# GEM3D/pressurePoissonSolver

Hardware: NVIDIA B200
Metric: fp64 GMG V-cycle DOF/s (higher is better)
Workload: dtype f64

## Files before the change

pressurepoissonsolver_b200/csrc/patch3d32.cuh:

```cuda
#pragma once

namespace tgpu
{
template <int D, int N, int MODE>
__device__ __forceinline__ double gamma_entry(const PatchMeta &pm, int p, int s, int m, const FaceVals<D, N, MODE> &fv)
{
	const int ty = pm.nbr_type[s];
	if (ty == NBR_NONE) return 0.0;
	if (ty == NBR_NORMAL) {
		const double a = fv.get(p, pm.parent_idx, pm.orth_on_parent, s, m);
		const double b = fv.get(pm.nbr_idx[s][0], pm.nbr_parent[s], pm.nbr_orth[s], s ^ 1, m);
		return 0.5 * a + 0.5 * b;
	}
	return iface_gamma<D, N, MODE>(pm, p, s, m, fv);
}

constexpr int    C32_THREADS = 512, C32_ROW = 34, C32_PL = 32 * C32_ROW, C32_TILE = 16 * C32_PL;
constexpr int    C32_FV = 65;
constexpr size_t smooth3d32c_smem_bytes() { return sizeof(double) * (C32_TILE + 2 * 1024 + 1024 + 16 * 128 + 16 * 64); }
static_assert(32 * C32_FV <= 1024 + 16 * 128, "the face-vector staging aliases the interface-value buffers of sweeps from a zero guess");
__device__ __forceinline__ unsigned cluster_ctarank()
{
	unsigned r;
	asm volatile("mov.u32 %0, %%cluster_ctarank;\n" : "=r"(r));
	return r;
}
__device__ __forceinline__ void cluster_sync_all()
{
	asm volatile("barrier.cluster.arrive.release.aligned;\nbarrier.cluster.wait.acquire.aligned;\n" ::: "memory");
}
__device__ __forceinline__ double ld_dsmem(const double *local, unsigned rank)
{
	unsigned a = (unsigned) __cvta_generic_to_shared(local), ra;
	double   v;
	asm volatile("mapa.shared::cluster.u32 %0, %1, %2;\n" : "=r"(ra) : "r"(a), "r"(rank));
	asm volatile("ld.shared::cluster.f64 %0, [%1];\n" : "=d"(v) : "r"(ra) : "memory");
	return v;
}
template <bool PROLONG>
__device__ __noinline__ double gamma_entry32(const PatchMeta *__restrict__ meta, int p, int s, int m, const double *__restrict__ F,
                                             const double *__restrict__ uc)
{
	const FaceVals<3, 32, PROLONG ? FV_PROLONG : FV_PLAIN> fv{F, uc, meta};
	return gamma_entry(meta[p], p, s, m, fv);
}
struct __align__(16) GDesc32 {
	unsigned a0, b0, a1, b1;
	double   c;
	int      flags, pad;
};
struct GPatch32 {
	GDesc32 d[6];
	int     neu, pad[3];
};
template <bool PROLONG>
__device__ __forceinline__ void make_gdesc32(const PatchMeta &pm, int p, int s, GPatch32 &out)
{
	GDesc32 & d  = out.d[s];
	const int ty = pm.nbr_type[s];
	const int ax = s >> 1;
	const int st = (ax == 0) ? 1 : (ax == 1 ? 32 : 1024);
	d.a0 = d.b0 = ((unsigned) p * 6 + s) * 1024;
	d.a1 = d.b1 = 0;
	d.c         = (ty == NBR_NONE) ? 0.0 : 2.0 * pm.inv_h2;
	int fl      = GD_SA | GD_SB | GD_WB;
	if (ty == NBR_NORMAL) {
		d.b0 = ((unsigned) pm.nbr_idx[s][0] * 6 + (s ^ 1)) * 1024;
		if (PROLONG) {
			const int o = pm.orth_on_parent, qp = pm.nbr_parent[s], qo = pm.nbr_orth[s];
			if (o >= 0) d.a1 = (unsigned) pm.parent_idx * 32768 + 16 * ((o & 1) + 32 * ((o >> 1) & 1) + 1024 * ((o >> 2) & 1)) + ((s & 1) ? 15 * st : 0);
			else d.a1 = (unsigned) pm.parent_idx * 32768 + ((s & 1) ? 31 * st : 0), fl &= ~GD_SA;
			if (qp < 0) d.b1 = d.a1, fl = (fl & ~(GD_SB | GD_WB)) | ((fl & GD_SA) ? GD_SB : 0);
			else if (qo >= 0) d.b1 = (unsigned) qp * 32768 + 16 * ((qo & 1) + 32 * ((qo >> 1) & 1) + 1024 * ((qo >> 2) & 1)) + ((s & 1) ? 0 : 15 * st);
			else d.b1 = (unsigned) qp * 32768 + ((s & 1) ? 0 : 31 * st), fl &= ~GD_SB;
		}
	} else if (ty > NBR_NORMAL) {
		fl = GD_SA | GD_SB | GD_WB | GD_SLOW;
	}
	d.flags = fl;
}
template <bool PROLONG> struct SideGamma32 {
	double a0, a1, b0, b1;
	template <int AX>
	__device__ __forceinline__ void issue(const GDesc32 &d, int m, int lo, int hi, const double *__restrict__ F, const double *__restrict__ uc)
	{
		constexpr int A = (AX == 0) ? 32 : 1, B = (AX == 2) ? 32 : 1024;
		const uint4   o = *reinterpret_cast<const uint4 *>(&d);
		a0 = __ldg(F + o.x + m);
		b0 = __ldg(F + o.y + m);
		a1 = b1 = 0.0;
		if (PROLONG) {
			const int fl = d.flags, sa = fl & GD_SA, sb = (fl >> 1) & 1;
			a1 = __ldg(uc + o.z + ((lo >> sa) * A + (hi >> sa) * B));
			b1 = __ldg(uc + o.w + ((lo >> sb) * A + (hi >> sb) * B));
		}
	}
	__device__ __forceinline__ double finish(const GDesc32 &d, const PatchMeta *__restrict__ meta, int p, int s, int m, const double *__restrict__ F,
	                                         const double *__restrict__ uc) const
	{
		const double c  = d.c;
		const int    fl = d.flags;
		double       g  = c * (0.5 * (a0 + a1) + 0.5 * (b0 + ((fl & GD_WB) ? b1 : 0.0)));
		if (fl & GD_SLOW) g = c * gamma_entry32<PROLONG>(meta, p, s, m, F, uc);
		return g;
	}
};

template <bool ZERO_GUESS, bool EMIT, bool PROLONG, bool WRITE_U, bool HALO = false>
__global__ void __cluster_dims__(2, 1, 1) __launch_bounds__(C32_THREADS, 1)
smooth3d32c_kernel(const PatchMeta *__restrict__ meta, int p0, int P, const double *__restrict__ f, double *__restrict__ u,
                   const double *__restrict__ Fin, double *__restrict__ Fout, const double *__restrict__ tri,
                   const double *__restrict__ uc, HaloSync hs = HaloSync{}, int skip_neumann = 0)
{
	constexpr int N = 32, ROW = C32_ROW, PL = C32_PL, M = N * N, NC = N * N * N;
	extern __shared__ __align__(16) double S[];
	double *       X    = S + C32_TILE;
	double *       GZ   = X + 2 * M;
	double *       GXY  = GZ + M;
	double *       EX   = GXY + 16 * 128;
	double *       FV   = GZ;
	const int      t = threadIdx.x, lane = t & 31, w = t >> 5;
	const unsigned rank = cluster_ctarank();
	const int      z    = rank == 0 ? w : N - 1 - w;
	const int      sz   = rank == 0 ? 4 : 5;
	const int      ncl = gridDim.x / 2, npatch = P - p0;
	double *       gxy  = GXY + w * 128;
	const int      mf   = lane + N * z;
	Mags<N>        mg;
	mg.load();
	pdl_launch_dependents();
	pdl_wait();
	if (!ZERO_GUESS) if (HALO) halo_push<3, 32>(hs, meta);
	int g = blockIdx.x / 2;
	bool halo_ok = false;
	constexpr int                   MW = (int) (sizeof(PatchMeta) / sizeof(double));
	__shared__ __align__(16) double metaS[MW];
	__shared__ GPatch32             GD[2];
	auto describe = [&](const PatchMeta &pm, int q, int slot) {
		if (lane == 31 && w < 6) make_gdesc32<PROLONG>(pm, q, w, GD[slot]);
		if (lane == 31 && w == 6) GD[slot].neu = pm.neumann;
	};
	const int zlo = t & 31, zhi = t >> 5;
	if (!ZERO_GUESS && g < npatch) {
		const int p = p0 + g;
		if (HALO) halo_wait_cta(hs, p, halo_ok);
		describe(meta[p], p, 0);
		if (g + ncl < npatch) describe(meta[p + ncl], p + ncl, 1);
		__syncthreads();
		SideGamma32<PROLONG> g6[6];
		g6[0].template issue<0>(GD[0].d[0], mf, lane, z, Fin, uc);
		g6[1].template issue<0>(GD[0].d[1], mf, lane, z, Fin, uc);
		g6[2].template issue<1>(GD[0].d[2], mf, lane, z, Fin, uc);
		g6[3].template issue<1>(GD[0].d[3], mf, lane, z, Fin, uc);
		g6[4].template issue<2>(GD[0].d[sz], t, zlo, zhi, Fin, uc);
		g6[5].template issue<2>(GD[0].d[sz], t + 512, zlo, zhi + 16, Fin, uc);
#pragma unroll
		for (int s = 0; s < 4; s++) gxy[s * 32 + lane] = g6[s].finish(GD[0].d[s], meta, p, s, mf, Fin, uc);
		GZ[t]       = g6[4].finish(GD[0].d[sz], meta, p, sz, t, Fin, uc);
		GZ[t + 512] = g6[5].finish(GD[0].d[sz], meta, p, sz, t + 512, Fin, uc);
		__syncthreads();
	}
	for (int it = 0; g < npatch; g += ncl, it++) {
		const int    p    = p0 + g;
		const bool   next = g + ncl < npatch;
		const int    pn   = p + ncl;
		const double h2   = meta[p].h2;
		double       v[N];
		if (!ZERO_GUESS && t < MW && g + 2 * ncl < npatch) cp_async8(&metaS[t], reinterpret_cast<const double *>(meta + pn + ncl) + t, true);
		if (skip_neumann && (ZERO_GUESS ? meta[p].neumann : GD[it & 1].neu)) {
			if (!ZERO_GUESS) {
				cp_async_wait_all();
				__syncthreads();
				const GPatch32 &gq = GD[(it + 1) & 1];
				if (next) {
					if (HALO) halo_wait_cta(hs, pn, halo_ok);
					SideGamma32<PROLONG> s6[6];
					s6[0].template issue<0>(gq.d[0], mf, lane, z, Fin, uc);
					s6[1].template issue<0>(gq.d[1], mf, lane, z, Fin, uc);
					s6[2].template issue<1>(gq.d[2], mf, lane, z, Fin, uc);
					s6[3].template issue<1>(gq.d[3], mf, lane, z, Fin, uc);
					s6[4].template issue<2>(gq.d[sz], t, zlo, zhi, Fin, uc);
					s6[5].template issue<2>(gq.d[sz], t + 512, zlo, zhi + 16, Fin, uc);
#pragma unroll
					for (int s = 0; s < 4; s++) gxy[s * 32 + lane] = s6[s].finish(gq.d[s], meta, pn, s, mf, Fin, uc);
					GZ[t]       = s6[4].finish(gq.d[sz], meta, pn, sz, t, Fin, uc);
					GZ[t + 512] = s6[5].finish(gq.d[sz], meta, pn, sz, t + 512, Fin, uc);
					if (g + 2 * ncl < npatch) describe(*reinterpret_cast<const PatchMeta *>(metaS), pn + ncl, it & 1);
				}
				__syncthreads();
			}
			cluster_sync_all();
			continue;
		}
		{
			const double *fp = f + (size_t) p * NC + (size_t) z * M + lane;
#pragma unroll
			for (int k = 0; k < N; k++) v[k] = __ldcs(fp + k * N);
			if (next) {
				const double *fn = f + (size_t) pn * NC + (size_t) z * M + lane * 32;
				prefetch_l2(fn);
				prefetch_l2(fn + 16);
			}
			if (!ZERO_GUESS) {
				v[0] -= gxy[64 + lane];
				v[N - 1] -= gxy[96 + lane];
				if (lane == 0 || lane == N - 1) {
					const double *q = gxy + (lane ? 32 : 0);
#pragma unroll
					for (int k = 0; k < N; k++) v[k] -= q[k];
				}
				if (w == 0) {
#pragma unroll
					for (int k = 0; k < N; k++) v[k] -= GZ[lane + N * k];
				}
			}
			Dst2<N, N>::run(v, mg);
			double *col = S + w * PL + lane;
#pragma unroll
			for (int k = 0; k < N; k++) col[k * ROW] = v[k];
		}
		__syncwarp();
		double2 *rowp = reinterpret_cast<double2 *>(S + w * PL + lane * ROW);
		{
#pragma unroll
			for (int j = 0; j < N / 2; j++) {
				const double2 d = rowp[j];
				v[2 * j]        = d.x;
				v[2 * j + 1]    = d.y;
			}
			Dst2<N, N>::run(v, mg);
#pragma unroll
			for (int j = 0; j < N / 2; j++) rowp[j] = make_double2(v[2 * j], v[2 * j + 1]);
		}
		if (!ZERO_GUESS) cp_async_wait_all();
		__syncthreads();
		if (HALO && !ZERO_GUESS && next) halo_wait_cta(hs, pn, halo_ok);
		SideGamma32<PROLONG> gm[3];
		const GPatch32 &     gp = GD[(it + 1) & 1];
		if (!ZERO_GUESS && next) {
			gm[0].template issue<0>(gp.d[0], mf, lane, z, Fin, uc);
			gm[1].template issue<0>(gp.d[1], mf, lane, z, Fin, uc);
			gm[2].template issue<1>(gp.d[2], mf, lane, z, Fin, uc);
			if (g + 2 * ncl < npatch) describe(*reinterpret_cast<const PatchMeta *>(metaS), pn + ncl, it & 1);
		}
		const double hsc = h2 * (4.0 / (N * N));
		double *     Xo = X + (it & 1) * M;
#pragma unroll
		for (int q = 0; q < 2; q++) {
			const int     ky = w + 16 * q;
			const double *zp = S + ky * ROW + lane;
			const double *tb = tri + ky * N + lane;
			double        rho = 0.0;
#pragma unroll
			for (int j = 0; j < 16; j++) {
				const double a = __ldg(tb + j * M);
				const double r = zp[j * PL] * (hsc * a);
				rho            = (j == 0) ? r : fma(-a, rho, r);
				const_cast<double *>(zp)[j * PL] = rho;
			}
			Xo[ky * N + lane] = rho;
		}
		if (!ZERO_GUESS && next) {
#pragma unroll
			for (int s = 0; s < 3; s++) gxy[s * 32 + lane] = gm[s].finish(gp.d[s], meta, pn, s, mf, Fin, uc);
			gm[0].template issue<1>(gp.d[3], mf, lane, z, Fin, uc);
			gm[1].template issue<2>(gp.d[sz], t, zlo, zhi, Fin, uc);
			gm[2].template issue<2>(gp.d[sz], t + 512, zlo, zhi + 16, Fin, uc);
		}
		cluster_sync_all();
#pragma unroll
		for (int q = 0; q < 2; q++) {
			const int     ky = w + 16 * q;
			double *      zp = S + ky * ROW + lane;
			const double *tb = tri + ky * N + lane;
			const double  a15 = __ldg(tb + 15 * M), kap = __ldg(tb + 16 * M);
			double        y   = kap * fma(-a15, ld_dsmem(Xo + ky * N + lane, rank ^ 1), zp[15 * PL]);
			zp[15 * PL]       = y;
#pragma unroll
			for (int j = 14; j >= 0; j--) {
				y          = fma(-__ldg(tb + j * M), y, zp[j * PL]);
				zp[j * PL] = y;
			}
		}
		if (!ZERO_GUESS && next) {
			gxy[96 + lane] = gm[0].finish(gp.d[3], meta, pn, 3, mf, Fin, uc);
			GZ[t]          = gm[1].finish(gp.d[sz], meta, pn, sz, t, Fin, uc);
			GZ[t + 512]    = gm[2].finish(gp.d[sz], meta, pn, sz, t + 512, Fin, uc);
		}
		__syncthreads();
		constexpr bool FACE_TAIL = ZERO_GUESS && !WRITE_U;
		if (!FACE_TAIL || w == 0) {
			{
#pragma unroll
				for (int j = 0; j < N / 2; j++) {
					const double2 d = rowp[j];
					v[2 * j]        = d.x;
					v[2 * j + 1]    = d.y;
				}
				Dst3<N, N>::run(v, mg);
#pragma unroll
				for (int j = 0; j < N / 2; j++) rowp[j] = make_double2(v[2 * j], v[2 * j + 1]);
			}
			__syncwarp();
			{
				const double *col = S + w * PL + lane;
#pragma unroll
				for (int k = 0; k < N; k++) v[k] = col[k * ROW];
				Dst3<N, N>::run(v, mg);
				if (WRITE_U) {
					double *up = u + (size_t) p * NC + (size_t) z * M + lane;
#pragma unroll
					for (int k = 0; k < N; k++) __stcs(up + k * N, v[k]);
				}
				if (EMIT) {
					double *Fp = Fout + (size_t) p * 6 * M;
					Fp[2 * M + mf] = v[0];
					Fp[3 * M + mf] = v[N - 1];
					if (w == 0) {
						double *Fz = Fp + sz * M + lane;
#pragma unroll
						for (int k = 0; k < N; k++) Fz[N * k] = v[k];
// ... 17 lines not shown
				E               = fma(mg.sinq(2 * j + 1), d.x, E);
				O               = fma((2 * j + 1 == N - 1) ? 0.5 : mg.sinq(2 * j + 2), d.y, O);
			}
			const int vi = 4 * (w - 1);
			FV[lane * C32_FV + vi]     = E + O;
			FV[lane * C32_FV + vi + 1] = E - O;
			const double *col = S + w * PL + lane;
			E = O = 0.0;
#pragma unroll
			for (int k = 0; k < N; k += 2) {
				E = fma(mg.sinq(k + 1), col[k * ROW], E);
				O = fma((k + 1 == N - 1) ? 0.5 : mg.sinq(k + 2), col[(k + 1) * ROW], O);
			}
			FV[lane * C32_FV + vi + 2] = E + O;
			FV[lane * C32_FV + vi + 3] = E - O;
		}
		if (FACE_TAIL) {
			__syncthreads();
			const int vec = (w - 1) * 32 + lane;
			if ((w == 1 || w == 2) && vec < 60) {
#pragma unroll
				for (int j = 0; j < N; j++) v[j] = FV[j * C32_FV + vec];
				Dst3<N, N>::run(v, mg);
				const int lp = 1 + (vec >> 2), kind = vec & 3;
				const int zz = rank == 0 ? lp : N - 1 - lp;
				double *  Fq = Fout + (size_t) p * 6 * M + kind * M + N * zz;
#pragma unroll
				for (int j = 0; j < N / 2; j++) *reinterpret_cast<double2 *>(Fq + 2 * j) = make_double2(v[2 * j], v[2 * j + 1]);
			}
		}
		__syncwarp();
	}
	cluster_sync_all();
	if (!ZERO_GUESS) if (HALO) halo_finish(hs);
}

__global__ void __launch_bounds__(TGPU_THREADS)
smooth3d32n_kernel(const PatchMeta *__restrict__ meta, int p0, int P, const double *__restrict__ f, double *__restrict__ u,
                   const double *__restrict__ Fin, double *__restrict__ Fout, const double *__restrict__ uc,
                   const double *__restrict__ mats, const double *__restrict__ lam, double *__restrict__ scratch, int zero_guess,
                   int emit, int prolong, int write_u, double lam_shift, int only_neumann = 0)
{
	constexpr int N = 32, M = N * N, NC = M * N;
	const int     t = threadIdx.x;
	double *      W = scratch + (size_t) blockIdx.x * NC;
	Mags<N>       mg;
	mg.load();
	pdl_launch_dependents();
	pdl_wait();
	for (int g = blockIdx.x; g < P - p0; g += gridDim.x) {
		const int        p    = p0 + g;
		const PatchMeta &pm   = meta[p];
		const int        neu  = pm.neumann;
		if (only_neumann && !neu) continue;
		const double     cfac = 2.0 * pm.inv_h2, h2 = pm.h2;
		for (int i = t; i < NC; i += TGPU_THREADS) W[i] = __ldg(f + (size_t) p * NC + i);
		__syncthreads();
		if (!zero_guess) {
			for (int s = 0; s < 6; s++) {
				if (pm.nbr_type[s] != NBR_NONE) {
					for (int m = t; m < M; m += TGPU_THREADS) {
						const double gm = prolong ? gamma_entry32<true>(meta, p, s, m, Fin, uc) : gamma_entry32<false>(meta, p, s, m, Fin, uc);
						int          c[3];
						face_cell<3, N>(s, m, c);
						W[(c[2] * N + c[1]) * N + c[0]] -= cfac * gm;
					}
				}
// ... 184 lines not shown
```

pressurepoissonsolver_b200/csrc/tgpu.cu:

```cuda
#include <algorithm>
#include <dlfcn.h>
#include <nccl.h>
#include <cmath>
#include <cstdio>
#include <cstdlib>
#include <cstring>
#include <map>
#include <memory>
#include <stdexcept>
#include <string>
#include <vector>

#include "../../include/tgpu.h"
#include "kernels.cuh"
#include "mesh.h"

using namespace tgpu;

extern "C" int tgpu_hierarchy_destroy(tgpu_hier *h);
static thread_local std::string g_last_error;
static int fail(int code, const std::string &msg)
{
	g_last_error = msg;
	return code;
// ... 125 lines not shown
}

struct tgpu_mesh {
	Mesh                       mesh;
	std::vector<HostLevel>     levels;
	std::vector<TgpuLevelDesc> descs;
};

struct tgpu_part {
	Partition                  part;
	std::vector<TgpuLevelDesc> descs;
};

struct PeerDev {
	int    peer = -1;
	size_t send_off = 0, send_n = 0, recv_off = 0, recv_n = 0;
};
struct LevelDev {
	int        P      = 0;
	int64_t    global_P = 0;
	int        slots  = 0;
	bool       distributed = false;
	int        n_interior  = 0;
	cudaEvent_t ev[4] = {nullptr, nullptr, nullptr, nullptr};
	std::vector<PeerDev> peers;
	int32_t *  send_patch = nullptr, *send_side = nullptr, *recv_slot = nullptr, *recv_side = nullptr;
	double *   sendbuf = nullptr, *recvbuf = nullptr;
	size_t     nsend = 0, nrecv = 0;
	size_t     ncells = 0, nface = 0;
	PatchMeta *meta    = nullptr;
	double *   starts  = nullptr;
	double *   spacing = nullptr;
	double *   Fa = nullptr, *Fb = nullptr;
	double *   u = nullptr, *f = nullptr, *r = nullptr;
	bool       has_neumann = false;
	int32_t *  neu_list = nullptr;
	std::vector<int32_t> neu_host;
	bool       p2p = false;
	int32_t *  send_peer = nullptr, *send_ridx = nullptr, *peer_rank = nullptr;
	double **  peerFa = nullptr, **peerFb = nullptr;
	uint64_t **peer_data_flag = nullptr, **peer_ack_flag = nullptr;
	uint64_t * data_flags = nullptr, *ack_flags = nullptr;
	uint64_t * cnt = nullptr;
	unsigned * tickets = nullptr;
	PushDesc * push_desc = nullptr;
	const double *push_uc = nullptr;
};

struct GraphEntry {
	bool    want_faces = false;
	double *faces      = nullptr;
	const double *  f;
	double *        u;
	TgpuCycleOpts   opts;
	cudaGraphExec_t exec;
	int64_t         kernels;
};

struct tgpu_hier {
	tgpu_ctx *            ctx = nullptr;
	int                   D = 0, N = 0;
	std::vector<LevelDev> levels;
	double *              scratch32 = nullptr;
	double *              cycle_faces = nullptr;
	double *              tri = nullptr;
	double *              mats = nullptr, *lam = nullptr;
// ... 121 lines not shown
}
static int set_smem_attrs_3d16()
{
	TRY((set_smem_attr_3d16<true, true, false, true>()));
	TRY((set_smem_attr_3d16<true, false, false, true>()));
	TRY((set_smem_attr_3d16<true, true, false, false>()));
	TRY((set_smem_attr_3d16<false, true, false, true>()));
	TRY((set_smem_attr_3d16<false, false, false, true>()));
	TRY((set_smem_attr_3d16<false, true, false, false>()));
	TRY((set_smem_attr_3d16<false, true, true, true>()));
	TRY((set_smem_attr_3d16<false, false, true, true>()));
	TRY((set_smem_attr_3d16<false, true, true, false>()));
	return TGPU_OK;
}
template <bool Z, bool E, bool PR, bool W> static int set_smem_attr_2d32()
{
	CU(cudaFuncSetAttribute(smooth2d32_kernel<Z, E, PR, W, false>, cudaFuncAttributeMaxDynamicSharedMemorySize, (int) smooth2d32_smem_bytes()));
	CU(cudaFuncSetAttribute(smooth2d32_kernel<Z, E, PR, W, true>, cudaFuncAttributeMaxDynamicSharedMemorySize, (int) smooth2d32_smem_bytes()));
	return TGPU_OK;
}
static int setup_2d32()
{
	TRY((set_smem_attr_2d32<true, true, false, true>()));
	TRY((set_smem_attr_2d32<true, false, false, true>()));
	TRY((set_smem_attr_2d32<true, true, false, false>()));
	TRY((set_smem_attr_2d32<false, true, false, true>()));
	TRY((set_smem_attr_2d32<false, false, false, true>()));
	TRY((set_smem_attr_2d32<false, true, false, false>()));
	TRY((set_smem_attr_2d32<false, true, true, true>()));
	TRY((set_smem_attr_2d32<false, false, true, true>()));
	TRY((set_smem_attr_2d32<false, true, true, false>()));
	return TGPU_OK;
}
template <bool Z, bool E, bool PR, bool W> static int set_smem_attr_3d32()
{
	CU(cudaFuncSetAttribute(smooth3d32c_kernel<Z, E, PR, W, !Z>, cudaFuncAttributeMaxDynamicSharedMemorySize, (int) smooth3d32c_smem_bytes()));
	return TGPU_OK;
}
static int setup_3d32(tgpu_hier *h)
{
	TRY((set_smem_attr_3d32<true, true, false, true>()));
	TRY((set_smem_attr_3d32<true, false, false, true>()));
	TRY((set_smem_attr_3d32<true, true, false, false>()));
	TRY((set_smem_attr_3d32<false, true, false, true>()));
	TRY((set_smem_attr_3d32<false, false, false, true>()));
	TRY((set_smem_attr_3d32<false, true, false, false>()));
	TRY((set_smem_attr_3d32<false, true, true, true>()));
	TRY((set_smem_attr_3d32<false, false, true, true>()));
	TRY((set_smem_attr_3d32<false, true, true, false>()));
	CU(cudaFuncSetAttribute(apply3d32_tma_kernel<0>, cudaFuncAttributeMaxDynamicSharedMemorySize, (int) apply3d32_tma_smem_bytes()));
	CU(cudaFuncSetAttribute(apply3d32_tma_kernel<1>, cudaFuncAttributeMaxDynamicSharedMemorySize, (int) apply3d32_tma_smem_bytes()));
	CU(cudaFuncSetAttribute(apply3d32_tma_kernel<3>, cudaFuncAttributeMaxDynamicSharedMemorySize, (int) apply3d32_tma_smem_bytes()));
	CU(cudaFuncSetAttribute(face_residual_restrict_big_kernel<3, 32, true>, cudaFuncAttributeMaxDynamicSharedMemorySize, 6 * 1024 * 8));
	CU(cudaFuncSetAttribute(face_residual_restrict_big_kernel<3, 32, false>, cudaFuncAttributeMaxDynamicSharedMemorySize, 6 * 1024 * 8));
	CU(cudaFuncSetAttribute(face_residual_restrict_big_kernel<3, 32, true, true>, cudaFuncAttributeMaxDynamicSharedMemorySize, 6 * 1024 * 8));
	CU(cudaFuncSetAttribute(face_residual_restrict_big_kernel<3, 32, false, true>, cudaFuncAttributeMaxDynamicSharedMemorySize, 6 * 1024 * 8));
	for (const LevelDev &L : h->levels)
		if (L.has_neumann && !h->scratch32) CU(cudaMalloc(&h->scratch32, (size_t) h->ctx->sm_count * 2 * 32768 * sizeof(double)));
	return TGPU_OK;
}
template <int D, int N> static int set_smem_attrs()
{
	const int sb = (int) smooth_smem_bytes<D, N, true>();
	CU(cudaFuncSetAttribute(smooth_kernel<D, N, true, true, false>, cudaFuncAttributeMaxDynamicSharedMemorySize, sb));
	CU(cudaFuncSetAttribute(smooth_kernel<D, N, true, false, false>, cudaFuncAttributeMaxDynamicSharedMemorySize, sb));
	CU(cudaFuncSetAttribute(smooth_kernel<D, N, false, true, false>, cudaFuncAttributeMaxDynamicSharedMemorySize, sb));
	CU(cudaFuncSetAttribute(smooth_kernel<D, N, false, false, false>, cudaFuncAttributeMaxDynamicSharedMemorySize, sb));
	CU(cudaFuncSetAttribute(smooth_kernel<D, N, false, true, true>, cudaFuncAttributeMaxDynamicSharedMemorySize, sb));
	CU(cudaFuncSetAttribute(smooth_kernel<D, N, false, false, true>, cudaFuncAttributeMaxDynamicSharedMemorySize, sb));
	if (D == 3 && N == 16) TRY(set_smem_attrs_3d16());
	CU(cudaFuncSetAttribute(apply_tma_kernel<D, N, 0>, cudaFuncAttributeMaxDynamicSharedMemorySize, (int) apply_tma_smem_bytes<D, N>()));
	CU(cudaFuncSetAttribute(apply_tma_kernel<D, N, 1>, cudaFuncAttributeMaxDynamicSharedMemorySize, (int) apply_tma_smem_bytes<D, N>()));
	CU(cudaFuncSetAttribute(apply_tma_kernel<D, N, 2>, cudaFuncAttributeMaxDynamicSharedMemorySize, (int) apply_tma_smem_bytes<D, N>()));
	CU(cudaFuncSetAttribute(apply_tma_kernel<D, N, 3>, cudaFuncAttributeMaxDynamicSharedMemorySize, (int) apply_tma_smem_bytes<D, N>()));
	return TGPU_OK;
}

static int init_constant_tables()
{
	for (int n : {4, 8, 16, 32}) {
		const int           H = n / 2;
		std::vector<double> fwd((size_t) n * H), inv((size_t) H * n);
// ... 321 lines not shown
		}
		for (size_t m = 0; m < M; m++) {
			const long double mu = (D == 2) ? ll[m] : ll[m % n] + ll[m / n];
			long double       a  = 0.0L;
			for (int j = 0; j < H; j++) {
				const long double d = mu - (j == 0 ? 3.0L : 2.0L);
				a                   = 1.0L / (d - (j == 0 ? 0.0L : a));
				tri[(size_t) j * M + m] = (double) a;
			}
			tri[(size_t) H * M + m] = (double) (1.0L / (1.0L - a * a));
		}
		TRY(dev_upload(&h->tri, tri.data(), tri.size()));
	}
	{
		std::vector<double> mats((size_t) 6 * n * n), lam((size_t) 3 * n);
		auto M = [&](int kind, int k, int j) -> double & { return mats[((size_t) kind * n + k) * n + j]; };
		for (int k = 0; k < n; k++)
			for (int j = 0; j < n; j++) {
				M(0, k, j) = sin(M_PI / n * ((k + 1) * (j + 0.5)));
				M(1, k, j) = (j == n - 1) ? ((k % 2 == 0) ? 0.5 : -0.5) : sin(M_PI / n * ((k + 0.5) * (j + 1)));
				M(2, k, j) = cos(M_PI / n * (k * (j + 0.5)));
				M(3, k, j) = (j == 0) ? 0.5 : cos(M_PI / n * ((k + 0.5) * j));
				M(4, k, j) = cos(M_PI / n * ((k + 0.5) * (j + 0.5)));
				M(5, k, j) = sin(M_PI / n * ((k + 0.5) * (j + 0.5)));
			}
		const double shift[3] = {1.0, 0.0, 0.5};
		for (int t = 0; t < 3; t++)
			for (int k = 0; k < n; k++) lam[(size_t) t * n + k] = -4.0 * pow(sin((k + shift[t]) * M_PI / (2 * n)), 2);
		TRY(dev_upload(&h->mats, mats.data(), mats.size()));
		TRY(dev_upload(&h->lam, lam.data(), lam.size()));
	}
	if (D == 3 && n == 32) TRY(setup_3d32(h.get()));
	else DISPATCH_DN(D, n, TRY((set_smem_attrs<DD, NN>())));
	if (D == 2 && n == 32) TRY(setup_2d32());
	*out = h.release();
	return TGPU_OK;
	API_END
}
extern "C" int tgpu_hierarchy_create(tgpu_ctx *ctx, int D, int n, int nlevels, const TgpuLevelDesc *levels, tgpu_hier **out)
{
	return hierarchy_create_impl(ctx, D, n, nlevels, levels, nullptr, out);
}

extern "C" int tgpu_mesh_partition(tgpu_mesh *m, int n, int rank, int nranks, int min_patches_per_rank, tgpu_part **out)
{
	API_BEGIN
	if (!m || !out) return fail(TGPU_ERR_ARG, "null argument");
	if (n < 2 || (n & 1)) return fail(TGPU_ERR_ARG, "n must be even and >= 2");
	std::unique_ptr<tgpu_part> p(new tgpu_part());
	std::vector<HostLevel>     global = m->mesh.extractLevels(n);
	p->part                           = partitionLevels(global, m->mesh.D, n, rank, nranks, min_patches_per_rank);
	for (const PartLevel &L : p->part.levels) p->descs.push_back(L.local.desc());
	*out = p.release();
	return TGPU_OK;
	API_END
}
extern "C" int tgpu_part_destroy(tgpu_part *p)
{
	delete p;
	return TGPU_OK;
}
extern "C" int tgpu_part_info(const tgpu_part *p, int *nlevels, int *ndist)
{
	if (!p) return fail(TGPU_ERR_ARG, "null partition");
	if (nlevels) *nlevels = (int) p->part.levels.size();
	if (ndist) *ndist = p->part.ndist;
// ... 306 lines not shown
	for (GraphEntry &g : h->graphs) cudaGraphExecDestroy(g.exec);
	h->graphs.clear();
}
extern "C" int tgpu_vec_destroy(tgpu_vec *v);
extern "C" int tgpu_hierarchy_destroy(tgpu_hier *h)
{
	if (!h) return TGPU_OK;
	cudaSetDevice(h->ctx->device);
	if (h->s_in) cudaStreamSynchronize(h->s_in);
	if (h->s_out) cudaStreamSynchronize(h->s_out);
	cudaStreamSynchronize(h->ctx->stream);
	free_graphs(h);
	for (tgpu_vec *v : h->krylov_ws) tgpu_vec_destroy(v);
	tgpu_vec_destroy(h->host_f);
	tgpu_vec_destroy(h->host_u);
	for (int k = 0; k < 2; k++) {
		tgpu_vec_destroy(h->pipe_f[k]);
		tgpu_vec_destroy(h->pipe_u[k]);
		if (h->ev_in[k]) cudaEventDestroy(h->ev_in[k]);
		if (h->ev_cyc[k]) cudaEventDestroy(h->ev_cyc[k]);
		if (h->ev_out[k]) cudaEventDestroy(h->ev_out[k]);
	}
	if (h->s_in) cudaStreamDestroy(h->s_in);
	if (h->s_out) cudaStreamDestroy(h->s_out);
	for (LevelDev &L : h->levels) {
		cudaFree(L.meta);
		cudaFree(L.neu_list);
		cudaFree(L.starts);
		cudaFree(L.spacing);
		if (!L.p2p) {
			cudaFree(L.Fa);
			cudaFree(L.Fb);
		}
		cudaFree(L.send_peer);
		cudaFree(L.send_ridx);
		cudaFree(L.peer_rank);
		cudaFree(L.peerFa);
		cudaFree(L.peerFb);
		cudaFree(L.peer_data_flag);
		cudaFree(L.peer_ack_flag);
		cudaFree(L.cnt);
		cudaFree(L.tickets);
		cudaFree(L.push_desc);
		for (int e = 0; e < 4; e++)
			if (L.ev[e]) cudaEventDestroy(L.ev[e]);
		cudaFree(L.send_patch);
		cudaFree(L.send_side);
		cudaFree(L.recv_slot);
		cudaFree(L.recv_side);
		cudaFree(L.sendbuf);
		cudaFree(L.recvbuf);
		cudaFree(L.u);
		cudaFree(L.f);
		cudaFree(L.r);
	}
	for (void *b : h->ipc_opened) cudaIpcCloseMemHandle(b);
	cudaFree(h->arena);
	cudaFree(h->p2p_abort);
	cudaFree(h->krylov_sc);
	cudaFree(h->mats);
	cudaFree(h->lam);
	cudaFree(h->scratch32);
	cudaFree(h->tri);
	delete h;
	return TGPU_OK;
}
// ... 8 lines not shown
	CU(cudaStreamSynchronize(ctx->stream));
	free_graphs(h);
	for (tgpu_vec *v : h->krylov_ws) tgpu_vec_destroy(v);
	h->krylov_ws.clear();
	tgpu_vec_destroy(h->host_f), h->host_f = nullptr;
	tgpu_vec_destroy(h->host_u), h->host_u = nullptr;
	for (int k = 0; k < 2; k++) {
		tgpu_vec_destroy(h->pipe_f[k]), h->pipe_f[k] = nullptr;
		tgpu_vec_destroy(h->pipe_u[k]), h->pipe_u[k] = nullptr;
	}
	h->pipe_count = 0;
	CU(cudaStreamSynchronize(ctx->stream));
	cudaMemPool_t pool = nullptr;
	CU(cudaDeviceGetDefaultMemPool(&pool, ctx->device));
	CU(cudaMemPoolTrimTo(pool, 0));
	return TGPU_OK;
	API_END
}
extern "C" int tgpu_hierarchy_info(const tgpu_hier *h, int *D, int *n, int *nlevels)
{
	if (!h) return fail(TGPU_ERR_ARG, "null hierarchy");
	if (D) *D = h->D;
	if (n) *n = h->N;
	if (nlevels) *nlevels = (int) h->levels.size();
	return TGPU_OK;
}
extern "C" int tgpu_hierarchy_set_lambda(tgpu_hier *h, double lambda)
{
	if (!h) return fail(TGPU_ERR_ARG, "null argument");
	if (!(lambda == lambda)) return fail(TGPU_ERR_ARG, "tgpu_hierarchy_set_lambda: lambda is NaN");
	h->lambda = lambda;
	if (lambda != 0.0 && is_3d32(h) && !h->scratch32) CU(cudaMalloc(&h->scratch32, (size_t) h->ctx->sm_count * 2 * 32768 * sizeof(double)));
	free_graphs(h);
	return TGPU_OK;
}
extern "C" int tgpu_hierarchy_force_generic_kernels(tgpu_hier *h, int on)
{
	if (!h) return fail(TGPU_ERR_ARG, "null argument");
	h->generic_kernels = on != 0;
	free_graphs(h);
	return TGPU_OK;
}
extern "C" int tgpu_level_npatch(const tgpu_hier *h, int level, int64_t *npatch, int64_t *ncells)
{
	if (!h || level < 0 || level >= (int) h->levels.size()) return fail(TGPU_ERR_ARG, "bad level");
	if (npatch) *npatch = h->levels[level].P;
	if (ncells) *ncells = (int64_t) h->levels[level].ncells;
	return TGPU_OK;
}

extern "C" int tgpu_vec_create(tgpu_hier *h, int level, tgpu_vec **out)
{
	if (!h || !out || level < 0 || level >= (int) h->levels.size()) return fail(TGPU_ERR_ARG, "tgpu_vec_create: bad argument");
	CU(cudaSetDevice(h->ctx->device));
	std::unique_ptr<tgpu_vec> v(new tgpu_vec());
	v->h     = h;
	v->level = level;
	v->n     = h->levels[level].ncells;
	CU(cudaMallocAsync(&v->d, std::max<size_t>(1, v->n) * sizeof(double), h->ctx->stream));
	CU(cudaMemsetAsync(v->d, 0, v->n * sizeof(double), h->ctx->stream));
	*out = v.release();
	return TGPU_OK;
}
extern "C" int tgpu_vec_destroy(tgpu_vec *v)
{
	if (!v) return TGPU_OK;
// ... 279 lines not shown
	if (p1 < 0) p1 = L.P;
	if (p1 <= p0) return hs.push ? fail(TGPU_ERR_ARG, "k_smooth: a launch that pushes faces needs patches") : TGPU_OK;
	if (!emit) write_u = true;
	struct ClampScope {
		tgpu_ctx *c;
		~ClampScope() { c->clamp_resident = false; }
	} clamp_scope{h->ctx};
	h->ctx->clamp_resident = hs.push != nullptr;
	Tag tg(h->ctx, zero_guess ? (write_u ? "smooth_zero_guess" : "smooth_zero_guess_faces")
	                          : (uc ? (write_u ? "smooth_prolong" : "smooth_prolong_faces") : (write_u ? "smooth" : "smooth_faces")),
	       l);
	const bool prolong = uc != nullptr;
	const PatchMeta *meta = L.meta;
	auto generic_smooth = [&](auto dd, auto nn, int only_neumann) {
		constexpr int DD = decltype(dd)::value, NN = decltype(nn)::value;
		using G          = Geo<DD, NN>;
		const int    nblk = (p1 - p0 + G::PPB - 1) / G::PPB;
		const dim3   grid(std::min(nblk, h->ctx->sm_count * smooth_min_blocks<NN>())), block(TGPU_THREADS);
		const size_t sm = smooth_smem_bytes<DD, NN, true>();
		return smooth_variant(zero_guess, emit, prolong, write_u, [&](auto Z, auto E, auto PR, auto) {
			return launch(h->ctx, smooth_kernel<DD, NN, Z, E, PR>, grid, block, sm, meta, p0, p1, f, u, Fin, Fout, (const double *) h->tri, uc,
			              (const double *) h->mats, (const double *) h->lam, h->lambda, only_neumann);
		});
	};
	const bool general = L.has_neumann || h->lambda != 0.0;
	const bool split = !(getenv("TGPU_NEUMANN_SPLIT") && atoi(getenv("TGPU_NEUMANN_SPLIT")) == 0);
	const bool mixed32 = is_3d32(h) && L.has_neumann && h->lambda == 0.0 && !hsp && split;
	if (is_3d32(h) && general) {
		const int nblk = std::min(p1 - p0, h->ctx->sm_count * 2);
		if (!h->scratch32) return fail(TGPU_ERR_ARG, "k_smooth: scratch for the general 32^3 patch solve missing");
		TRY(launch(h->ctx, smooth3d32n_kernel, dim3(nblk), dim3(TGPU_THREADS), 0, (const PatchMeta *) L.meta, p0, p1, f, u, Fin, Fout, uc,
		           (const double *) h->mats, (const double *) h->lam, h->scratch32, (int) zero_guess, (int) emit, (int) (uc != nullptr), (int) write_u, h->lambda,
		           mixed32 ? 1 : 0));
		if (!mixed32) return TGPU_OK;
	}
	if (is_3d32(h)) {
		const dim3   grid(2 * std::min(p1 - p0, h->ctx->sm_count / 2)), block(C32_THREADS);
		const size_t sm    = smooth3d32c_smem_bytes();
		const int    skipn = mixed32 ? 1 : 0;
		return smooth_variant(zero_guess, emit, prolong, write_u, [&](auto Z, auto E, auto PR, auto W) {
			return launch(h->ctx, smooth3d32c_kernel<Z, E, PR, W, !Z>, grid, block, sm, meta, p0, p1, f, u, Fin, Fout, (const double *) h->tri, uc, hs, skipn);
		});
	}
	const bool mixed16 = h->D == 3 && h->N == 16 && !h->generic_kernels && L.has_neumann && h->lambda == 0.0 && !hsp && split;
	if (h->D == 3 && h->N == 16 && !h->generic_kernels && (!general || mixed16)) {
		const int skipn = mixed16 ? 1 : 0;
		static const bool neu_fast = !(getenv("TGPU_NEUMANN_FAST") && atoi(getenv("TGPU_NEUMANN_FAST")) == 0);
		if (mixed16 && neu_fast) {
			TRY(smooth_variant(zero_guess, emit, prolong, write_u, [&](auto Z, auto E, auto PR, auto W) {
				return launch_smooth3d16<Z, E, PR, W>(h, L, p0, p1, f, u, Fin, Fout, uc, HaloSync{}, 0, true);
			}));
		} else if (mixed16) {
			TRY(generic_smooth(std::integral_constant<int, 3>{}, std::integral_constant<int, 16>{}, 1));
		}
		return smooth_variant(zero_guess, emit, prolong, write_u, [&](auto Z, auto E, auto PR, auto W) {
			return launch_smooth3d16<Z, E, PR, W>(h, L, p0, p1, f, u, Fin, Fout, uc, hs, skipn);
		});
	}
	const bool mixed2d = h->D == 2 && h->N == 32 && !h->generic_kernels && L.has_neumann && h->lambda == 0.0 && !hsp && split;
	if (mixed2d)
		TRY(generic_smooth(std::integral_constant<int, 2>{}, std::integral_constant<int, 32>{}, 1));
	if (h->D == 2 && h->N == 32 && !h->generic_kernels && (!general || mixed2d)) {
		const int    nblk = (p1 - p0 + Q32_WARPS - 1) / Q32_WARPS;
		const dim3   grid(std::min(nblk, h->ctx->sm_count * 2)), block(TGPU_THREADS);
		const size_t sm    = smooth2d32_smem_bytes();
		const int    skipn = mixed2d ? 1 : 0;
		return smooth_variant(zero_guess, emit, prolong, write_u, [&](auto Z, auto E, auto PR, auto W) {
			if (skipn || hs.enabled) return launch(h->ctx, smooth2d32_kernel<Z, E, PR, W, true>, grid, block, sm, meta, p0, p1, f, u, Fin, Fout, (const double *) h->tri, uc, hs, skipn);
			return launch(h->ctx, smooth2d32_kernel<Z, E, PR, W, false>, grid, block, sm, meta, p0, p1, f, u, Fin, Fout, (const double *) h->tri, uc, hs, skipn);
		});
	}
	DISPATCH_DN(h->D, h->N, return generic_smooth(std::integral_constant<int, DD>{}, std::integral_constant<int, NN>{}, 0));
}
static int k_face_residual_restrict(tgpu_hier *h, int l, const double *Fnew, const double *Fold, double *coarse, int p0 = 0, int p1 = -1,
// ... 828 lines not shown
```

Measured before the change: 81.31 billion.

## Split 32^3 interface-term gathering into a separate pre-transformed RHS kernel

Moves the gathering of interface gamma values out of the clustered 32^3 smoother into a new iface_rhs32 kernel. That kernel computes the six face terms per patch, applies the DST in the face-parallel directions and writes them to a per-level G buffer. The smoother then subtracts these pre-transformed values at the matching stage of its separable transform, instead of gathering and pipelining neighbour face values itself. This takes the irregular gathers and their shared-memory staging off the smoother's critical path and frees shared memory for the non-zero-guess variant. In exchange it adds a kernel launch, a global round trip through G, and extra device memory per level.

```diff
diff --git a/pressurepoissonsolver_b200/csrc/patch3d32.cuh b/pressurepoissonsolver_b200/csrc/patch3d32.cuh
--- a/pressurepoissonsolver_b200/csrc/patch3d32.cuh
+++ b/pressurepoissonsolver_b200/csrc/patch3d32.cuh
@@ -17,8 +17,11 @@
 
 constexpr int    C32_THREADS = 512, C32_ROW = 34, C32_PL = 32 * C32_ROW, C32_TILE = 16 * C32_PL;
 constexpr int    C32_FV = 65;
-constexpr size_t smooth3d32c_smem_bytes() { return sizeof(double) * (C32_TILE + 2 * 1024 + 1024 + 16 * 128 + 16 * 64); }
-static_assert(32 * C32_FV <= 1024 + 16 * 128, "the face-vector staging aliases the interface-value buffers of sweeps from a zero guess");
+template <bool ZERO_GUESS> constexpr size_t smooth3d32c_smem_bytes()
+{
+	return sizeof(double) * (C32_TILE + 2 * 1024 + 16 * 64 + (ZERO_GUESS ? 1024 + 16 * 128 : 0));
+}
+static_assert(32 * C32_FV <= 1024 + 16 * 128, "the face-vector staging of sweeps from a zero guess");
 __device__ __forceinline__ unsigned cluster_ctarank()
 {
 	unsigned r;
@@ -51,7 +54,6 @@
 };
 struct GPatch32 {
 	GDesc32 d[6];
-	int     neu, pad[3];
 };
 template <bool PROLONG>
 __device__ __forceinline__ void make_gdesc32(const PatchMeta &pm, int p, int s, GPatch32 &out)
@@ -95,102 +97,146 @@
 			b1 = __ldg(uc + o.w + ((lo >> sb) * A + (hi >> sb) * B));
 		}
 	}
+	__device__ __forceinline__ double combine(const GDesc32 &d) const
+	{
+		return d.c * (0.5 * (a0 + a1) + 0.5 * (b0 + ((d.flags & GD_WB) ? b1 : 0.0)));
+	}
 	__device__ __forceinline__ double finish(const GDesc32 &d, const PatchMeta *__restrict__ meta, int p, int s, int m, const double *__restrict__ F,
 	                                         const double *__restrict__ uc) const
 	{
-		const double c  = d.c;
-		const int    fl = d.flags;
-		double       g  = c * (0.5 * (a0 + a1) + 0.5 * (b0 + ((fl & GD_WB) ? b1 : 0.0)));
-		if (fl & GD_SLOW) g = c * gamma_entry32<PROLONG>(meta, p, s, m, F, uc);
+		double g = combine(d);
+		if (d.flags & GD_SLOW) g = d.c * gamma_entry32<PROLONG>(meta, p, s, m, F, uc);
 		return g;
 	}
 };
 
-template <bool ZERO_GUESS, bool EMIT, bool PROLONG, bool WRITE_U, bool HALO = false>
+constexpr int    IR32_THREADS = 192, IR32_CTAS_PER_SM = 2, IR32_TP = 33;
+constexpr size_t iface_rhs32_smem_bytes() { return sizeof(double) * 6 * 32 * IR32_TP; }
+constexpr int IR32_BATCH = 16;
+template <bool PROLONG, int AX>
+__device__ __forceinline__ void side_gamma32(const GDesc32 &d, const PatchMeta *__restrict__ meta, int p, int s, int lane, const double *__restrict__ F,
+                                             const double *__restrict__ uc, double *out, int stride)
+{
+	if (d.flags & GD_SLOW) {
+#pragma unroll 1
+		for (int i = 0; i < 32; i++) {
+			SideGamma32<PROLONG> sg;
+			sg.template issue<AX>(d, lane + 32 * i, lane, i, F, uc);
+			out[i * stride + lane] = sg.finish(d, meta, p, s, lane + 32 * i, F, uc);
+		}
+		return;
+	}
+	constexpr int B = IR32_BATCH;
+#pragma unroll
+	for (int i0 = 0; i0 < 32; i0 += B) {
+		SideGamma32<PROLONG> sg[B];
+#pragma unroll
+		for (int j = 0; j < B; j++) sg[j].template issue<AX>(d, lane + 32 * (i0 + j), lane, i0 + j, F, uc);
+#pragma unroll
+		for (int j = 0; j < B; j++) out[(i0 + j) * stride + lane] = sg[j].combine(d);
+	}
+}
+template <bool PROLONG, bool HALO>
+__global__ void __launch_bounds__(IR32_THREADS, IR32_CTAS_PER_SM)
+iface_rhs32_kernel(const PatchMeta *__restrict__ meta, int p0, int P, const double *__restrict__ Fin, const double *__restrict__ uc,
+                   double *__restrict__ Gout, HaloSync hs = HaloSync{}, int skip_neumann = 0)
+{
+	constexpr int N = 32, M = N * N, TP = IR32_TP;
+	extern __shared__ __align__(16) double T[];
+	__shared__ GPatch32 GD;
+	const int lane = threadIdx.x & 31, s = threadIdx.x >> 5;
+	double *  tw   = T + s * N * TP;
+	Mags<N>   mg;
+	mg.load();
+	pdl_launch_dependents();
+	pdl_wait();
+	if (HALO) halo_push<3, 32>(hs, meta);
+	bool halo_ok = false;
+	for (int g = blockIdx.x; g < P - p0; g += gridDim.x) {
+		const int p = p0 + g;
+		if (skip_neumann && meta[p].neumann) continue;
+		if (HALO) halo_wait_cta(hs, p, halo_ok);
+		if (lane == 0) make_gdesc32<PROLONG>(meta[p], p, s, GD);
+		__syncwarp();
+		const GDesc32 &d  = GD.d[s];
+		double *       Gp = Gout + ((size_t) p * 6 + s) * M;
+		double         v[N];
+		if (s < 2) {
+			side_gamma32<PROLONG, 0>(d, meta, p, s, lane, Fin, uc, tw, TP);
+			__syncwarp();
+#pragma unroll
+			for (int k = 0; k < N; k++) v[k] = tw[lane * TP + k];
+			Dst2<N, N>::run(v, mg);
+#pragma unroll
+			for (int k = 0; k < N; k++) tw[lane * TP + k] = v[k];
+			__syncwarp();
+#pragma unroll
+			for (int i = 0; i < N; i++) Gp[lane + N * i] = tw[i * TP + lane];
+		} else if (s < 4) {
+			side_gamma32<PROLONG, 1>(d, meta, p, s, lane, Fin, uc, Gp, N);
+		} else {
+			side_gamma32<PROLONG, 2>(d, meta, p, s, lane, Fin, uc, tw, TP);
+			__syncwarp();
+#pragma unroll
+			for (int k = 0; k < N; k++) v[k] = tw[k * TP + lane];
+			Dst2<N, N>::run(v, mg);
+#pragma unroll
+			for (int k = 0; k < N; k++) tw[k * TP + lane] = v[k];
+			__syncwarp();
+#pragma unroll
+			for (int k = 0; k < N; k++) v[k] = tw[lane * TP + k];
+			Dst2<N, N>::run(v, mg);
+#pragma unroll
+			for (int k = 0; k < N; k++) tw[lane * TP + k] = v[k];
+			__syncwarp();
+#pragma unroll
+			for (int i = 0; i < N; i++) Gp[lane + N * i] = tw[i * TP + lane];
+		}
+		__syncwarp();
+	}
+	if (HALO) halo_finish(hs);
+}
+
+template <bool ZERO_GUESS, bool EMIT, bool WRITE_U>
 __global__ void __cluster_dims__(2, 1, 1) __launch_bounds__(C32_THREADS, 1)
 smooth3d32c_kernel(const PatchMeta *__restrict__ meta, int p0, int P, const double *__restrict__ f, double *__restrict__ u,
-                   const double *__restrict__ Fin, double *__restrict__ Fout, const double *__restrict__ tri,
-                   const double *__restrict__ uc, HaloSync hs = HaloSync{}, int skip_neumann = 0)
+                   const double *__restrict__ G, double *__restrict__ Fout, const double *__restrict__ tri, int skip_neumann = 0)
 {
 	constexpr int N = 32, ROW = C32_ROW, PL = C32_PL, M = N * N, NC = N * N * N;
 	extern __shared__ __align__(16) double S[];
 	double *       X    = S + C32_TILE;
-	double *       GZ   = X + 2 * M;
-	double *       GXY  = GZ + M;
-	double *       EX   = GXY + 16 * 128;
-	double *       FV   = GZ;
+	double *       FV   = X + 2 * M;
+	double *       EX   = FV + (ZERO_GUESS ? 1024 + 16 * 128 : 0);
 	const int      t = threadIdx.x, lane = t & 31, w = t >> 5;
 	const unsigned rank = cluster_ctarank();
 	const int      z    = rank == 0 ? w : N - 1 - w;
 	const int      sz   = rank == 0 ? 4 : 5;
 	const int      ncl = gridDim.x / 2, npatch = P - p0;
-	double *       gxy  = GXY + w * 128;
 	const int      mf   = lane + N * z;
 	Mags<N>        mg;
 	mg.load();
 	pdl_launch_dependents();
 	pdl_wait();
-	if (!ZERO_GUESS) if (HALO) halo_push<3, 32>(hs, meta);
 	int g = blockIdx.x / 2;
-	bool halo_ok = false;
-	constexpr int                   MW = (int) (sizeof(PatchMeta) / sizeof(double));
-	__shared__ __align__(16) double metaS[MW];
-	__shared__ GPatch32             GD[2];
-	auto describe = [&](const PatchMeta &pm, int q, int slot) {
-		if (lane == 31 && w < 6) make_gdesc32<PROLONG>(pm, q, w, GD[slot]);
-		if (lane == 31 && w == 6) GD[slot].neu = pm.neumann;
-	};
-	const int zlo = t & 31, zhi = t >> 5;
-	if (!ZERO_GUESS && g < npatch) {
-		const int p = p0 + g;
-		if (HALO) halo_wait_cta(hs, p, halo_ok);
-		describe(meta[p], p, 0);
-		if (g + ncl < npatch) describe(meta[p + ncl], p + ncl, 1);
-		__syncthreads();
-		SideGamma32<PROLONG> g6[6];
-		g6[0].template issue<0>(GD[0].d[0], mf, lane, z, Fin, uc);
-		g6[1].template issue<0>(GD[0].d[1], mf, lane, z, Fin, uc);
-		g6[2].template issue<1>(GD[0].d[2], mf, lane, z, Fin, uc);
-		g6[3].template issue<1>(GD[0].d[3], mf, lane, z, Fin, uc);
-		g6[4].template issue<2>(GD[0].d[sz], t, zlo, zhi, Fin, uc);
-		g6[5].template issue<2>(GD[0].d[sz], t + 512, zlo, zhi + 16, Fin, uc);
-#pragma unroll
-		for (int s = 0; s < 4; s++) gxy[s * 32 + lane] = g6[s].finish(GD[0].d[s], meta, p, s, mf, Fin, uc);
-		GZ[t]       = g6[4].finish(GD[0].d[sz], meta, p, sz, t, Fin, uc);
-		GZ[t + 512] = g6[5].finish(GD[0].d[sz], meta, p, sz, t + 512, Fin, uc);
-		__syncthreads();
-	}
 	for (int it = 0; g < npatch; g += ncl, it++) {
 		const int    p    = p0 + g;
 		const bool   next = g + ncl < npatch;
 		const int    pn   = p + ncl;
 		const double h2   = meta[p].h2;
 		double       v[N];
-		if (!ZERO_GUESS && t < MW && g + 2 * ncl < npatch) cp_async8(&metaS[t], reinterpret_cast<const double *>(meta + pn + ncl) + t, true);
-		if (skip_neumann && (ZERO_GUESS ? meta[p].neumann : GD[it & 1].neu)) {
-			if (!ZERO_GUESS) {
-				cp_async_wait_all();
-				__syncthreads();
-				const GPatch32 &gq = GD[(it + 1) & 1];
-				if (next) {
-					if (HALO) halo_wait_cta(hs, pn, halo_ok);
-					SideGamma32<PROLONG> s6[6];
-					s6[0].template issue<0>(gq.d[0], mf, lane, z, Fin, uc);
-					s6[1].template issue<0>(gq.d[1], mf, lane, z, Fin, uc);
-					s6[2].template issue<1>(gq.d[2], mf, lane, z, Fin, uc);
-					s6[3].template issue<1>(gq.d[3], mf, lane, z, Fin, uc);
-					s6[4].template issue<2>(gq.d[sz], t, zlo, zhi, Fin, uc);
-					s6[5].template issue<2>(gq.d[sz], t + 512, zlo, zhi + 16, Fin, uc);
-#pragma unroll
-					for (int s = 0; s < 4; s++) gxy[s * 32 + lane] = s6[s].finish(gq.d[s], meta, pn, s, mf, Fin, uc);
-					GZ[t]       = s6[4].finish(gq.d[sz], meta, pn, sz, t, Fin, uc);
-					GZ[t + 512] = s6[5].finish(gq.d[sz], meta, pn, sz, t + 512, Fin, uc);
-					if (g + 2 * ncl < npatch) describe(*reinterpret_cast<const PatchMeta *>(metaS), pn + ncl, it & 1);
-				}
-				__syncthreads();
-			}
+		if (skip_neumann && meta[p].neumann) {
 			cluster_sync_all();
 			continue;
+		}
+		double gy0 = 0.0, gy1 = 0.0, gx0 = 0.0, gx1 = 0.0, gz0 = 0.0, gz1 = 0.0;
+		if (!ZERO_GUESS) {
+			const double *Gp = G + (size_t) p * 6 * M;
+			gy0              = __ldcs(Gp + 2 * M + mf);
+			gy1              = __ldcs(Gp + 3 * M + mf);
+			gx0              = __ldcs(Gp + 0 * M + mf);
+			gx1              = __ldcs(Gp + 1 * M + mf);
+			gz0              = __ldcs(Gp + sz * M + lane + N * w);
+			gz1              = __ldcs(Gp + sz * M + lane + N * (w + 16));
 		}
 		{
 			const double *fp = f + (size_t) p * NC + (size_t) z * M + lane;
@@ -200,19 +246,14 @@
 				const double *fn = f + (size_t) pn * NC + (size_t) z * M + lane * 32;
 				prefetch_l2(fn);
 				prefetch_l2(fn + 16);
+				if (!ZERO_GUESS && lane < 12) {
+					const double *Gn = G + (size_t) pn * 6 * M + 16 * (lane & 1);
+					prefetch_l2(lane < 8 ? Gn + (lane >> 1) * M + N * z : Gn + sz * M + N * (w + 16 * ((lane >> 1) & 1)));
+				}
 			}
 			if (!ZERO_GUESS) {
-				v[0] -= gxy[64 + lane];
-				v[N - 1] -= gxy[96 + lane];
-				if (lane == 0 || lane == N - 1) {
-					const double *q = gxy + (lane ? 32 : 0);
-#pragma unroll
-					for (int k = 0; k < N; k++) v[k] -= q[k];
-				}
-				if (w == 0) {
-#pragma unroll
-					for (int k = 0; k < N; k++) v[k] -= GZ[lane + N * k];
-				}
+				v[0] -= gy0;
+				v[N - 1] -= gy1;
 			}
 			Dst2<N, N>::run(v, mg);
 			double *col = S + w * PL + lane;
@@ -228,21 +269,15 @@
 				v[2 * j]        = d.x;
 				v[2 * j + 1]    = d.y;
 			}
+			if (!ZERO_GUESS) {
+				v[0] -= gx0;
+				v[N - 1] -= gx1;
+			}
 			Dst2<N, N>::run(v, mg);
 #pragma unroll
 			for (int j = 0; j < N / 2; j++) rowp[j] = make_double2(v[2 * j], v[2 * j + 1]);
 		}
-		if (!ZERO_GUESS) cp_async_wait_all();
 		__syncthreads();
-		if (HALO && !ZERO_GUESS && next) halo_wait_cta(hs, pn, halo_ok);
-		SideGamma32<PROLONG> gm[3];
-		const GPatch32 &     gp = GD[(it + 1) & 1];
-		if (!ZERO_GUESS && next) {
-			gm[0].template issue<0>(gp.d[0], mf, lane, z, Fin, uc);
-			gm[1].template issue<0>(gp.d[1], mf, lane, z, Fin, uc);
-			gm[2].template issue<1>(gp.d[2], mf, lane, z, Fin, uc);
-			if (g + 2 * ncl < npatch) describe(*reinterpret_cast<const PatchMeta *>(metaS), pn + ncl, it & 1);
-		}
 		const double hsc = h2 * (4.0 / (N * N));
 		double *     Xo = X + (it & 1) * M;
 #pragma unroll
@@ -254,18 +289,12 @@
 #pragma unroll
 			for (int j = 0; j < 16; j++) {
 				const double a = __ldg(tb + j * M);
-				const double r = zp[j * PL] * (hsc * a);
+				const double x = (!ZERO_GUESS && j == 0) ? zp[0] - (q ? gz1 : gz0) : zp[j * PL];
+				const double r = x * (hsc * a);
 				rho            = (j == 0) ? r : fma(-a, rho, r);
 				const_cast<double *>(zp)[j * PL] = rho;
 			}
 			Xo[ky * N + lane] = rho;
-		}
-		if (!ZERO_GUESS && next) {
-#pragma unroll
-			for (int s = 0; s < 3; s++) gxy[s * 32 + lane] = gm[s].finish(gp.d[s], meta, pn, s, mf, Fin, uc);
-			gm[0].template issue<1>(gp.d[3], mf, lane, z, Fin, uc);
-			gm[1].template issue<2>(gp.d[sz], t, zlo, zhi, Fin, uc);
-			gm[2].template issue<2>(gp.d[sz], t + 512, zlo, zhi + 16, Fin, uc);
 		}
 		cluster_sync_all();
 #pragma unroll
@@ -282,11 +311,6 @@
 				zp[j * PL] = y;
 			}
 		}
-		if (!ZERO_GUESS && next) {
-			gxy[96 + lane] = gm[0].finish(gp.d[3], meta, pn, 3, mf, Fin, uc);
-			GZ[t]          = gm[1].finish(gp.d[sz], meta, pn, sz, t, Fin, uc);
-			GZ[t + 512]    = gm[2].finish(gp.d[sz], meta, pn, sz, t + 512, Fin, uc);
-		}
 		__syncthreads();
 		constexpr bool FACE_TAIL = ZERO_GUESS && !WRITE_U;
 		if (!FACE_TAIL || w == 0) {
@@ -370,7 +394,6 @@
 		__syncwarp();
 	}
 	cluster_sync_all();
-	if (!ZERO_GUESS) if (HALO) halo_finish(hs);
 }
 
 __global__ void __launch_bounds__(TGPU_THREADS)
diff --git a/pressurepoissonsolver_b200/csrc/tgpu.cu b/pressurepoissonsolver_b200/csrc/tgpu.cu
--- a/pressurepoissonsolver_b200/csrc/tgpu.cu
+++ b/pressurepoissonsolver_b200/csrc/tgpu.cu
@@ -181,6 +181,7 @@
 	double *   starts  = nullptr;
 	double *   spacing = nullptr;
 	double *   Fa = nullptr, *Fb = nullptr;
+	double *   G  = nullptr;
 	double *   u = nullptr, *f = nullptr, *r = nullptr;
 	bool       has_neumann = false;
 	int32_t *  neu_list = nullptr;
@@ -368,22 +369,37 @@
 	TRY((set_smem_attr_2d32<false, true, true, false>()));
 	return TGPU_OK;
 }
-template <bool Z, bool E, bool PR, bool W> static int set_smem_attr_3d32()
-{
-	CU(cudaFuncSetAttribute(smooth3d32c_kernel<Z, E, PR, W, !Z>, cudaFuncAttributeMaxDynamicSharedMemorySize, (int) smooth3d32c_smem_bytes()));
+template <bool Z, bool E, bool W> static int set_smem_attr_3d32()
+{
+	CU(cudaFuncSetAttribute(smooth3d32c_kernel<Z, E, W>, cudaFuncAttributeMaxDynamicSharedMemorySize, (int) smooth3d32c_smem_bytes<Z>()));
+	return TGPU_OK;
+}
+static int update_iface_buffers(tgpu_hier *h)
+{
+	if (!is_3d32(h)) return TGPU_OK;
+	for (LevelDev &L : h->levels) {
+		const bool want = h->lambda == 0.0 && L.neu_host.size() < (size_t) L.P;
+		if (want && !L.G) CU(cudaMalloc(&L.G, (size_t) L.P * 6 * 1024 * sizeof(double)));
+		if (!want && L.G) {
+			CU(cudaDeviceSynchronize());
+			cudaFree(L.G);
+			L.G = nullptr;
+		}
+	}
 	return TGPU_OK;
 }
 static int setup_3d32(tgpu_hier *h)
 {
-	TRY((set_smem_attr_3d32<true, true, false, true>()));
-	TRY((set_smem_attr_3d32<true, false, false, true>()));
-	TRY((set_smem_attr_3d32<true, true, false, false>()));
-	TRY((set_smem_attr_3d32<false, true, false, true>()));
-	TRY((set_smem_attr_3d32<false, false, false, true>()));
-	TRY((set_smem_attr_3d32<false, true, false, false>()));
-	TRY((set_smem_attr_3d32<false, true, true, true>()));
-	TRY((set_smem_attr_3d32<false, false, true, true>()));
-	TRY((set_smem_attr_3d32<false, true, true, false>()));
+	TRY((set_smem_attr_3d32<true, true, true>()));
+	TRY((set_smem_attr_3d32<true, false, true>()));
+	TRY((set_smem_attr_3d32<true, true, false>()));
+	TRY((set_smem_attr_3d32<false, true, true>()));
+	TRY((set_smem_attr_3d32<false, false, true>()));
+	TRY((set_smem_attr_3d32<false, true, false>()));
+	CU(cudaFuncSetAttribute(iface_rhs32_kernel<false, false>, cudaFuncAttributeMaxDynamicSharedMemorySize, (int) iface_rhs32_smem_bytes()));
+	CU(cudaFuncSetAttribute(iface_rhs32_kernel<true, false>, cudaFuncAttributeMaxDynamicSharedMemorySize, (int) iface_rhs32_smem_bytes()));
+	CU(cudaFuncSetAttribute(iface_rhs32_kernel<false, true>, cudaFuncAttributeMaxDynamicSharedMemorySize, (int) iface_rhs32_smem_bytes()));
+	CU(cudaFuncSetAttribute(iface_rhs32_kernel<true, true>, cudaFuncAttributeMaxDynamicSharedMemorySize, (int) iface_rhs32_smem_bytes()));
 	CU(cudaFuncSetAttribute(apply3d32_tma_kernel<0>, cudaFuncAttributeMaxDynamicSharedMemorySize, (int) apply3d32_tma_smem_bytes()));
 	CU(cudaFuncSetAttribute(apply3d32_tma_kernel<1>, cudaFuncAttributeMaxDynamicSharedMemorySize, (int) apply3d32_tma_smem_bytes()));
 	CU(cudaFuncSetAttribute(apply3d32_tma_kernel<3>, cudaFuncAttributeMaxDynamicSharedMemorySize, (int) apply3d32_tma_smem_bytes()));
@@ -771,6 +787,7 @@
 	}
 	if (D == 3 && n == 32) TRY(setup_3d32(h.get()));
 	else DISPATCH_DN(D, n, TRY((set_smem_attrs<DD, NN>())));
+	TRY(update_iface_buffers(h.get()));
 	if (D == 2 && n == 32) TRY(setup_2d32());
 	*out = h.release();
 	return TGPU_OK;
@@ -1143,6 +1160,7 @@
 			cudaFree(L.Fa);
 			cudaFree(L.Fb);
 		}
+		cudaFree(L.G);
 		cudaFree(L.send_peer);
 		cudaFree(L.send_ridx);
 		cudaFree(L.peer_rank);
@@ -1217,6 +1235,7 @@
 	h->lambda = lambda;
 	if (lambda != 0.0 && is_3d32(h) && !h->scratch32) CU(cudaMalloc(&h->scratch32, (size_t) h->ctx->sm_count * 2 * 32768 * sizeof(double)));
 	free_graphs(h);
+	TRY(update_iface_buffers(h));
 	return TGPU_OK;
 }
 extern "C" int tgpu_hierarchy_force_generic_kernels(tgpu_hier *h, int on)
@@ -1562,14 +1581,26 @@
 		TRY(launch(h->ctx, smooth3d32n_kernel, dim3(nblk), dim3(TGPU_THREADS), 0, (const PatchMeta *) L.meta, p0, p1, f, u, Fin, Fout, uc,
 		           (const double *) h->mats, (const double *) h->lam, h->scratch32, (int) zero_guess, (int) emit, (int) (uc != nullptr), (int) write_u, h->lambda,
 		           mixed32 ? 1 : 0));
-		if (!mixed32) return TGPU_OK;
+		if (!mixed32 || L.neu_host.size() == (size_t) L.P) return TGPU_OK;
 	}
 	if (is_3d32(h)) {
-		const dim3   grid(2 * std::min(p1 - p0, h->ctx->sm_count / 2)), block(C32_THREADS);
-		const size_t sm    = smooth3d32c_smem_bytes();
-		const int    skipn = mixed32 ? 1 : 0;
-		return smooth_variant(zero_guess, emit, prolong, write_u, [&](auto Z, auto E, auto PR, auto W) {
-			return launch(h->ctx, smooth3d32c_kernel<Z, E, PR, W, !Z>, grid, block, sm, meta, p0, p1, f, u, Fin, Fout, (const double *) h->tri, uc, hs, skipn);
+		const int skipn = mixed32 ? 1 : 0;
+		if (!zero_guess) {
+			if (!L.G) return fail(TGPU_ERR_ARG, "k_smooth: interface-term buffer of the 32^3 level missing");
+			Tag          ti(h->ctx, "iface_rhs", l);
+			const dim3   gi(std::min(p1 - p0, h->ctx->sm_count * IR32_CTAS_PER_SM)), bi(IR32_THREADS);
+			const size_t si = iface_rhs32_smem_bytes();
+			if (hs.enabled && prolong) TRY(launch(h->ctx, iface_rhs32_kernel<true, true>, gi, bi, si, meta, p0, p1, Fin, uc, L.G, hs, skipn));
+			else if (hs.enabled) TRY(launch(h->ctx, iface_rhs32_kernel<false, true>, gi, bi, si, meta, p0, p1, Fin, uc, L.G, hs, skipn));
+			else if (prolong) TRY(launch(h->ctx, iface_rhs32_kernel<true, false>, gi, bi, si, meta, p0, p1, Fin, uc, L.G, hs, skipn));
+			else TRY(launch(h->ctx, iface_rhs32_kernel<false, false>, gi, bi, si, meta, p0, p1, Fin, uc, L.G, hs, skipn));
+		} else if (hs.enabled) {
+			return fail(TGPU_ERR_ARG, "smooth3d32c: no halo hand-over in a zero-guess sweep");
+		}
+		const dim3 grid(2 * std::min(p1 - p0, h->ctx->sm_count / 2)), block(C32_THREADS);
+		return smooth_variant(zero_guess, emit, prolong, write_u, [&](auto Z, auto E, auto, auto W) {
+			return launch(h->ctx, smooth3d32c_kernel<Z, E, W>, grid, block, smooth3d32c_smem_bytes<Z>(), meta, p0, p1, f, u,
+			              (const double *) L.G, Fout, (const double *) h->tri, skipn);
 		});
 	}
 	const bool mixed16 = h->D == 3 && h->N == 16 && !h->generic_kernels && L.has_neumann && h->lambda == 0.0 && !hsp && split;
```

Result: faster. 86.07 billion, median of 6 (+5.9%).
